# OpenDrift/opendrift

Hardware: AMD Instinct MI355X
Metric: particle-steps/sec (RK4, 3D interp) (higher is better)
Workload: dtype f64; 1 GPU; C3: OceanDrift 3D, synthetic ROMS-shaped z-level grid 1024x1024x12 (u,v,w,K), RK4 + vertical_mixing(60 s) + vertical_advection; particles_per_gpu=10000000, particles_total=10000000, stage_math=fast, spin_up_steps=200, block_every=0, inputs=resident in HBM, parallelism=particle-sharded x1, field block broadcast once per time level

## Files before the change

opendrift_amd/csrc/odr_kernels.hip.h:

```cpp
#pragma once
#include <hip/hip_runtime.h>
#include <rocrand/rocrand_kernel.h>
#include "odr_field.hip.h"

namespace odr {

#ifndef ODR_BLOCK
#define ODR_BLOCK 256
#endif
constexpr int BLOCK = ODR_BLOCK;
#ifndef ODR_POLAR_WAVES
#define ODR_POLAR_WAVES 3
#endif
#ifndef ODR_POLAR_STEP_WAVES
#define ODR_POLAR_STEP_WAVES 2
#endif
#define ODR_STEP_WAVES(PROJ) ((PROJ) == PROJ_LATLONG ? ODR_LATLONG_WAVES : ((PROJ) == PROJ_EXT ? 1 : ODR_POLAR_STEP_WAVES))
#ifndef ODR_LATLONG_WAVES
#define ODR_LATLONG_WAVES 1
#endif
#define ODR_WAVES(PROJ) ((PROJ) == PROJ_LATLONG ? ODR_LATLONG_WAVES : ((PROJ) == PROJ_EXT ? 1 : ODR_POLAR_WAVES))

__device__ __forceinline__ long long pid() {
  const unsigned nb = gridDim.x, b = blockIdx.x, per = nb >> 3, rem = nb & 7u, x = b & 7u, j = b >> 3;
// ... 259 lines not shown
    r.x = rad * ((kq == 2u || kq == 3u) ? -s1 : s1);
    r.y = rad * ((kq == 1u || kq == 2u) ? -c1 : c1);
  }
  return r;
#endif
}

constexpr unsigned long long RNG_OFF_NOISE_UNIFORM = 64, RNG_OFF_NOISE_STAGE = 128;
struct StageNoise {
  int on, rng_mode, ncomp;
  int sm;
  double std_n, std_u;
  const double *main, *stage;
  unsigned long long seed, step;
};
__device__ __forceinline__ void add_f32_f64(float &u, float &v, double nx, double ny) {
  u = (float)__dadd_rn((double)u, nx);
  v = (float)__dadd_rn((double)v, ny);
}
__device__ __forceinline__ void add_current_noise(const StageNoise &N, int call, long long i, long long n, int id,
                                                  float &u, float &v) {
  if (N.rng_mode == 1) {
    const double *a = call == 0 ? N.main : N.stage + (size_t)(call - 1) * (size_t)N.ncomp * (size_t)n;
    int c = 0;
    if (N.std_n > 0) { add_f32_f64(u, v, a[i], a[(size_t)n + i]); c = 2; }
    if (N.std_u > 0) add_f32_f64(u, v, a[(size_t)c * (size_t)n + i], a[(size_t)(c + 1) * (size_t)n + i]);
  } else {
    const unsigned long long off = RNG_OFF_NOISE + (call == 0 ? 4ull * (unsigned)VAR_U : RNG_OFF_NOISE_STAGE + 8ull * (unsigned)call);
    if (N.std_n > 0) {
      const double2 g = rng_normal2(rng_block(N.seed, id, N.step, off));
      add_f32_f64(u, v, g.x * N.std_n, g.y * N.std_n);
    }
    if (N.std_u > 0) {
      const double2 q = rng_uniform2(rng_block(N.seed, id, N.step, off + (call == 0 ? RNG_OFF_NOISE_UNIFORM : 4ull)));
      add_f32_f64(u, v, fma(2.0 * N.std_u, q.x, -N.std_u), fma(2.0 * N.std_u, q.y, -N.std_u));
    }
  }
}

#ifndef ODR_MIX_ROUNDS
#define ODR_MIX_ROUNDS 10
#endif
template <int ROUNDS>
__device__ __forceinline__ uint4 philox4x32(uint4 c, unsigned k0, unsigned k1) {
#pragma unroll
  for (int r = 0; r < ROUNDS; ++r) {
    const unsigned long long p0 = (unsigned long long)0xD2511F53u * c.x, p1 = (unsigned long long)0xCD9E8D57u * c.z;
    c = make_uint4((unsigned)(p1 >> 32) ^ c.y ^ k0, (unsigned)p1, (unsigned)(p0 >> 32) ^ c.w ^ k1, (unsigned)p0);
    k0 += 0x9E3779B9u; k1 += 0xBB67AE85u;
  }
  return c;
}
struct MixKey { unsigned k0, k1, step_lo, tag, id; };
__device__ __forceinline__ MixKey mix_key(unsigned long long seed, unsigned long long step, int id) {
  MixKey K;
  K.k0 = (unsigned)seed; K.k1 = (unsigned)(seed >> 32);
  K.step_lo = (unsigned)step; K.tag = 0x4D495856u ^ (unsigned)(step >> 32); K.id = (unsigned)id;
  return K;
}
__device__ __forceinline__ uint4 mix_block(const MixKey &K, unsigned b) {
  return philox4x32<ODR_MIX_ROUNDS>(make_uint4(b, K.step_lo, K.id, K.tag), K.k0, K.k1);
}
__device__ __forceinline__ unsigned mix_word(const uint4 &q, unsigned k) {
  const unsigned lo = ((q.x & 255u) << 16) | ((q.y & 255u) << 8) | (q.z & 255u);
  return k == 0 ? q.x >> 8 : (k == 1 ? q.y >> 8 : (k == 2 ? q.z >> 8 : (k == 3 ? q.w >> 8 : lo)));
}
__device__ __forceinline__ unsigned mix_draw(const MixKey &K, uint4 &q, int it, bool primed = false) {
  const unsigned b = (unsigned)it / 5u, k = (unsigned)it - 5u * b;
  if (k == 0 && !(primed && it == 0)) q = mix_block(K, b);
  return mix_word(q, k);
}
__device__ __forceinline__ double mix_uniform(const MixKey &K, uint4 &q, int it, bool primed = false) {
  return ((double)mix_draw(K, q, it, primed) + 0.5) * 5.9604644775390625e-08;
}
__device__ __forceinline__ double mix_R_of(unsigned x) {
  return (double)((int)(2u * x + 1u) - (1 << 24)) * 5.9604644775390625e-08;
}
constexpr int AUX_KMEMBER = 8;
struct VMixDesc {
  int sid, nzp, geo_slot;
  unsigned kstride;
  const float *kb, *ka;
  double wgt;
  float Kfb, pad2;
  const unsigned long long *guard;
};

struct VMixRT {
  static constexpr bool STATIC = false;
  __host__ __device__ static constexpr int proj_kind(int k) { return k; }
  __host__ __device__ static constexpr int lon_mode(int m) { return m; }
  __host__ __device__ static constexpr int mod360_x(int m) { return m; }
  __host__ __device__ static constexpr int nzp(int n, int ) { return n; }
  __host__ __device__ static constexpr bool uniform_z(bool u) { return u; }
  __host__ __device__ static constexpr int rng_mode(int m) { return m; }
  __host__ __device__ static constexpr int mix_at_surface(int m) { return m; }
  __host__ __device__ static constexpr int sf_action(int a) { return a; }
  __host__ __device__ static constexpr int vadv(int v) { return v; }
  __host__ __device__ static constexpr int ntimes(int n) { return n; }
  __host__ __device__ static constexpr unsigned kstride(unsigned b, int ) { return b; }
  __device__ static void proj_fwd(const DevProj &p, double lon, double lat, double &x, double &y) { proj_fwd_rt(p, lon, lat, x, y); }
};
struct VMixC3 {
  static constexpr bool STATIC = true;
  __host__ __device__ static constexpr int proj_kind(int) { return PROJ_LATLONG; }
  __host__ __device__ static constexpr int lon_mode(int) { return 1; }
  __host__ __device__ static constexpr int mod360_x(int) { return 0; }
  __host__ __device__ static constexpr int nzp(int, int NL) { return NL; }
  __host__ __device__ static constexpr bool uniform_z(bool) { return false; }
  __host__ __device__ static constexpr int rng_mode(int) { return 0; }
  __host__ __device__ static constexpr int mix_at_surface(int) { return 0; }
  __host__ __device__ static constexpr int sf_action(int) { return 1; }
  __host__ __device__ static constexpr int vadv(int) { return 0; }
  __host__ __device__ static constexpr int ntimes(int) { return 10; }
  __host__ __device__ static constexpr unsigned kstride(unsigned, int NQ) { return 16u * (unsigned)NQ; }
  __device__ static void proj_fwd(const DevProj &, double lon, double lat, double &x, double &y) { x = lon; y = lat; }
};

struct VMixC3Rec : VMixC3 {
  __host__ __device__ static constexpr unsigned kstride(unsigned b, int ) { return b; }
};

template <int NQ, bool TL, class VM, class HOOK>
__device__ __forceinline__ void vmix_col_fill(const DevSource &s, const VMixDesc &D, double lon, double lat, double *Kp,
                                              int tid, HOOK &&hook) {
  const double Kfb = (double)D.Kfb;
  double x, y;
  const int lon_mode = VM::lon_mode(s.lon_mode);
  if (lon_mode == 1) lon = np_mod(lon + 180.0, 360.0) - 180.0;
  else if (lon_mode == 2) lon = np_mod(lon, 360.0);
  VM::proj_fwd(s.proj, lon, lat, x, y);
  const bool cov = x >= s.xmin && x <= s.xmax && y >= s.ymin && y <= s.ymax;
  if (VM::mod360_x(s.mod360_x)) x = np_mod(x, 360.0);
  const DevBlock &bb = s.slot[D.geo_slot];
  const double xi = __dmul_rn(div_cr(x - bb.x0, bb.xspan, bb.ixspan), (double)(bb.nx - 1));
  const double yi = __dmul_rn(div_cr(y - bb.y0, bb.yspan, bb.iyspan), (double)(bb.ny - 1));
  const int ny = bb.ny, nx = bb.nx;
  const Axis ay = axis_fp(yi, ny), ax = axis_fp(xi, nx);
  const double ty = ay.t, tx = ax.t, wy0 = 1 - ty, wx0 = 1 - tx, wgt = D.wgt;
  const unsigned recb = VM::kstride(D.kstride, NQ);
  const unsigned r0 = __umul24((unsigned)ay.i0, (unsigned)nx), r1 = __umul24((unsigned)ay.i1, (unsigned)nx);
  const unsigned o00 = cov ? __umul24(r0 + (unsigned)ax.i0, recb) : 0u, o01 = cov ? __umul24(r0 + (unsigned)ax.i1, recb) : 0u;
  const unsigned o10 = cov ? __umul24(r1 + (unsigned)ax.i0, recb) : 0u, o11 = cov ? __umul24(r1 + (unsigned)ax.i1, recb) : 0u;
  const float *kb = D.kb, *ka = TL ? D.ka : D.kb;
  const double w00 = wy0 * wx0, w01 = wy0 * tx, w10 = ty * wx0, w11 = ty * tx;
#pragma unroll
  for (int q = 0; q < NQ; ++q) {
    if (VM::STATIC && q > 0) __builtin_amdgcn_sched_barrier(0);
    const F4 b00 = ld_off<F4>(kb, o00 + 16u * q), b01 = ld_off<F4>(kb, o01 + 16u * q);
    const F4 b10 = ld_off<F4>(kb, o10 + 16u * q), b11 = ld_off<F4>(kb, o11 + 16u * q);
    F4 a00, a01, a10, a11;
    if (TL) {
      a00 = ld_off<F4>(ka, o00 + 16u * q); a01 = ld_off<F4>(ka, o01 + 16u * q);
      a10 = ld_off<F4>(ka, o10 + 16u * q); a11 = ld_off<F4>(ka, o11 + 16u * q);
    }
    if (VM::STATIC && q > 0) __builtin_amdgcn_sched_barrier(0);
    if (q == 0) hook();
    double v[4];
    v[0] = (double)bilw(b00.x, b01.x, b10.x, b11.x, w00, w01, w10, w11);
    v[1] = (double)bilw(b00.y, b01.y, b10.y, b11.y, w00, w01, w10, w11);
    v[2] = (double)bilw(b00.z, b01.z, b10.z, b11.z, w00, w01, w10, w11);
    v[3] = (double)bilw(b00.w, b01.w, b10.w, b11.w, w00, w01, w10, w11);
    if (TL) {
      double w[4];
      w[0] = (double)bilw(a00.x, a01.x, a10.x, a11.x, w00, w01, w10, w11);
      w[1] = (double)bilw(a00.y, a01.y, a10.y, a11.y, w00, w01, w10, w11);
      w[2] = (double)bilw(a00.z, a01.z, a10.z, a11.z, w00, w01, w10, w11);
      w[3] = (double)bilw(a00.w, a01.w, a10.w, a11.w, w00, w01, w10, w11);
#pragma unroll
      for (int j = 0; j < 4; ++j) v[j] = __dadd_rn(__dmul_rn(v[j], 1 - wgt), __dmul_rn(w[j], wgt));
    }
#pragma unroll
    for (int j = 0; j < 4; ++j) Kp[(4 * q + j) * BLOCK + tid] = (cov && isfinite(v[j])) ? v[j] : Kfb;
  }
}

struct VMixArgs {
  double dt, dt_mix_cfg;
  int mix_at_surface, rng_mode, sfl, pad;
  const double *huni;
  unsigned long long seed, step;
};
struct MixRng { MixKey key; uint4 q; bool primed; };
template <class VM = VMixRT>
__device__ __forceinline__ MixRng mix_rng_begin(const VMixArgs &A, int id) {
  MixRng R;
  R.key = mix_key(A.seed, A.step, id);
  R.q = make_uint4(0u, 0u, 0u, 0u);
  R.primed = false;
  if (VM::rng_mode(A.rng_mode) == 0) {
    R.q = mix_block(R.key, 0u);
    R.primed = true;
  }
  return R;
}
template <int NQ, class VM = VMixRT>
__device__ __forceinline__ double vmix_col_walk(const DevSource &s, int nzp, const double *Kp, const double *gsh, int tid,
                                                const VMixArgs &A, long long i, long long n, int id, double z, int &moving,
                                                float Zmin, float tv, int &sf_flags, const MixRng *pre) {
  constexpr int NL = 4 * NQ;
  static_assert(!VM::STATIC || NL >= 3, "a static configuration has the three-level window inside the profile");
  const double dt = A.dt;
  const int mix_at_surface = VM::mix_at_surface(A.mix_at_surface), rng_mode = VM::rng_mode(A.rng_mode), sfl = A.sfl;
  double zm[NL - 1];
#pragma unroll
  for (int k = 0; k < NL - 1; ++k) zm[k] = k < nzp - 1 ? s.zmid[k] : __builtin_inf();
  const bool uniform_z = VM::uniform_z(s.vg_uniform != 0);
  const double gd0 = s.vg_d[0], gi0 = s.vg_id[0], gd1 = s.vg_d[1], gi1 = s.vg_id[1], gd2 = s.vg_d[2], gi2 = s.vg_id[2];
  const double sgn = dt > 0 ? 1.0 : (dt < 0 ? -1.0 : 0.0);
  const double dt_mix = A.dt_mix_cfg * sgn;
  const int ntimes = VM::ntimes(abs((int)(dt / dt_mix)));
  const double r = 1.0 / 3, ir = 1.0 / r;
  double wstep = __dmul_rn(__dmul_rn((double)tv, dt_mix), (double)moving);
  const MixKey st = mix_key(A.seed, A.step, id);
  uint4 u4 = make_uint4(0u, 0u, 0u, 0u);
  bool primed = false;
  if (pre) { u4 = pre->q; primed = pre->primed; }
  auto level_terms = [&](auto edges, int zl, double &dk_dt, double &sg) {
    constexpr int E = decltype(edges)::value;
    const double Kz = Kp[zl * BLOCK + tid];
    double gK;
    if ((E & 1) && zl == 0) gK = div_cr(Kp[BLOCK + tid] - Kz, gd0, gi0);
    else if ((E & 2) && zl == nzp - 1) gK = div_cr(Kz - Kp[(nzp - 2) * BLOCK + tid], gd1, gi1);
    else if (uniform_z) gK = div_cr(Kp[(zl + 1) * BLOCK + tid] - Kp[(zl - 1) * BLOCK + tid], gd2, gi2);
    else
      gK = __dadd_rn(__dadd_rn(__dmul_rn(gsh[zl], Kp[(zl - 1) * BLOCK + tid]), __dmul_rn(gsh[NL + zl], Kz)),
                     __dmul_rn(gsh[2 * NL + zl], Kp[(zl + 1) * BLOCK + tid]));
    double dK = -gK;
    if (fabs(dK) < 1e-10) dK = 0;
    dk_dt = __dmul_rn(dK, dt_mix);
    sg = sqrt(div_cr(__dmul_rn(__dmul_rn(Kz, fabs(dt_mix)), 2.0), r, ir));
  };
  using AnyLevel = std::integral_constant<int, 3>;
  int lv0;
  {
    const double d0 = -z;
    int zs = 0;
#pragma unroll
    for (int k = 0; k < NL - 1; ++k) zs += ((k & 1) ? d0 >= zm[k] : d0 > zm[k]) ? 1 : 0;
    lv0 = zs < 1 ? 1 : (zs > nzp - 2 ? nzp - 2 : zs);
    if (nzp < 3) lv0 = 1;
  }
  double c_dk[3], c_sg[3];
#pragma unroll
  for (int q = 0; q < 3; ++q) {
    const int zl = lv0 - 1 + q;
    c_dk[q] = 0; c_sg[q] = 0;
    if constexpr (VM::STATIC) {
      if (q == 0) level_terms(std::integral_constant<int, 1>(), zl, c_dk[q], c_sg[q]);
      else if (q == 1) level_terms(std::integral_constant<int, 0>(), zl, c_dk[q], c_sg[q]);
      else level_terms(std::integral_constant<int, 2>(), zl, c_dk[q], c_sg[q]);
    } else if (zl >= 0 && zl < nzp) level_terms(AnyLevel(), zl, c_dk[q], c_sg[q]);
  }
  double wb[4];
#pragma unroll
  for (int j = 0; j < 4; ++j) {
    const int k = lv0 - 2 + j;
    double b = k < 0 ? -1.0 : __builtin_inf();
    if (k >= 0 && k < nzp - 1) {
      b = gsh[3 * NL + k];
      if ((k & 1) && b > 0) b = __longlong_as_double(__double_as_longlong(b) - 1);
    }
    wb[j] = b;
  }
  for (int it0 = 0; it0 < ntimes; it0 += 5) {
  if (rng_mode == 0 && !(primed && it0 == 0)) u4 = mix_block(st, (unsigned)it0 / 5u);
#pragma unroll
  for (int k5 = 0; k5 < 5; ++k5) {
    const int it = it0 + k5;
    if (it >= ntimes) break;
    const bool surface = z == 0;
    const double d = -z;
    int q = (d > wb[1] ? 1 : 0) + (d > wb[2] ? 1 : 0);
    int zi = lv0 - 1 + q;
    if (!(d > wb[0]) || d > wb[3]) {
      zi = 0;
#pragma unroll
      for (int k = 0; k < NL - 1; ++k) zi += ((k & 1) ? d >= zm[k] : d > zm[k]) ? 1 : 0;
      q = zi - lv0 + 1;
    }
    double dKdt = q == 0 ? c_dk[0] : (q == 1 ? c_dk[1] : c_dk[2]);
    double sig = q == 0 ? c_sg[0] : (q == 1 ? c_sg[1] : c_sg[2]);
    if (q < 0 || q > 2) level_terms(AnyLevel(), zi, dKdt, sig);
    double R;
    if (rng_mode == 1) R = __dsub_rn(__dmul_rn(2.0, A.huni[(size_t)it * n + i]), 1.0);
    else R = mix_R_of(mix_word(u4, (unsigned)k5));
    z = __dsub_rn(z, __dmul_rn((double)moving, __dsub_rn(dKdt, __dmul_rn(R, sig))));
    if (z >= 0) z = -z;
    if (z < (double)Zmin && moving == 1) z = __dsub_rn((double)__fmul_rn(2.f, Zmin), z);
    z = __dadd_rn(z, wstep);
    if (!mix_at_surface && surface) z = 0.0;
    if (z > 0) z = 0.0;
    if (z < (double)Zmin) {
      const int act = VM::sf_action(sfl & 255);
      if (act == 3) sf_flags |= 2;
      else if (act) {
        z = (double)Zmin;
        if (act == 2) { sf_flags |= 1; moving = 0; wstep = 0.0; }
        else if (act == 4) { sf_flags |= 4; moving = 0; wstep = 0.0; }
        else if (act == 5 && (sf_flags & 8)) { sf_flags |= 4; moving = 0; wstep = 0.0; }
      }
    }
  }
  }
  return z;
}

__device__ __forceinline__ float pick_slot(const float (&a)[MAXG], int j) {
  float r = a[0];
#pragma unroll
  for (int k = 1; k < MAXG; ++k) {
    float v = a[k];
    asm volatile("" : "+v"(v));
    r = j == k ? v : r;
  }
  return r;
}

#ifdef ODR_TU_MISC
template <int NV>
struct GroupVars { int v[NV]; };

template <int NV>
__global__ __launch_bounds__(BLOCK) void k_env_group(const DevWorld *__restrict__ W, PView p,
                                                     GroupVars<NV> gv, double t, int record_prev) {
  long long i = (long long)blockIdx.x * BLOCK + threadIdx.x;
  if (i >= p.n) return;
  int vars[NV];
#pragma unroll
  for (int k = 0; k < NV; ++k) vars[k] = gv.v[k];
  double lon = p.lon[i], lat = p.lat[i], z = p.z[i];
  float out[NV];
  env_group<NV>(*W, vars, lon, lat, z, t, out, p.rank ? p.rank[i] : 0, W->f32pos & 1);
#pragma unroll
  for (int k = 0; k < NV; ++k) p.env[vars[k]][i] = out[k];
  if (record_prev) { p.slon[i] = lon; p.slat[i] = lat; }
}

template <int PROJ>
__global__ __launch_bounds__(BLOCK, ODR_WAVES(PROJ)) void k_env_grid(const DevWorld *__restrict__ W, PView p, EnvGroupDesc G,
                                                    int record_prev) {
  long long i = pid();
  if (i >= p.n) return;
  double lon = p.lon[i], lat = p.lat[i], z = p.z[i];
  int f32idx = 0;
  if (W->f32pos & 1) {
    lon = lon_f32class(W->src[G.sid].lon_mode, lon);
    if (PROJ == PROJ_LATLONG) f32idx = W->src[G.sid].xy_f32;
  }
  float out[MAXG];
  env_group_fast<PROJ>(*W, G, lon, lat, z, out, f32idx);
#pragma unroll
  for (int k = 0; k < MAXG; ++k)
    if (k < G.nv) G.out_ptr[k][i] = out[k];
  if (record_prev) { p.slon[i] = lon; p.slat[i] = lat; }
}

__global__ __launch_bounds__(BLOCK) void k_fill_f32(float *a, long long n, float v) {
  long long i = (long long)blockIdx.x * BLOCK + threadIdx.x;
  if (i < n) a[i] = v;
}

__global__ __launch_bounds__(BLOCK) void k_record_prev(PView p, int which) {
  long long i = (long long)blockIdx.x * BLOCK + threadIdx.x;
  if (i >= p.n) return;
  if (which == 0) { p.slon[i] = p.lon[i]; p.slat[i] = p.lat[i]; }
  else { p.plon[i] = p.lon[i]; p.plat[i] = p.lat[i]; }
}

#endif
#ifdef ODR_TU_STEP
__device__ __forceinline__ float rk4_mix(float k1, float k2, float k3, float k4) {
  float s = __fadd_rn(k1, __fmul_rn(2.0f, k2));
  s = __fadd_rn(s, __fmul_rn(2.0f, k3));
  s = __fadd_rn(s, k4);
  return div_cr_f32(s, 6.0f, 1.0f / 6.0f);
}

template <int SCHEME, bool NOISE>
__global__ __launch_bounds__(BLOCK) void k_advect(const DevWorld *__restrict__ W, PView p, double t,
                                                  double dt, float factor, StageNoise N) {
  long long i = (long long)blockIdx.x * BLOCK + threadIdx.x;
  if (i >= p.n) return;
  const int uv[2] = {VAR_U, VAR_V};
  double lon = p.lon[i], lat = p.lat[i], z = p.z[i];
  float u1 = p.env[VAR_U][i], v1 = p.env[VAR_V][i];
// ... 917 lines not shown
        zi += ((k & 1) ? d >= mid : d > mid) ? 1 : 0;
      }
    if (zi != zi_cur) {
      zi_cur = zi;
      const double Kz = Kp[zi * BLOCK + tid];
      double gK = 0;
      if (nzp >= 2) {
        if (zi == 0) gK = div_cr(Kp[BLOCK + tid] - Kz, src->vg_d[0], src->vg_id[0]);
        else if (zi == nzp - 1) {
          if (nzp == nz_full) gK = div_cr(Kz - Kp[(nzp - 2) * BLOCK + tid], src->vg_d[1], src->vg_id[1]);
          else gK = __ddiv_rn(Kz - Kp[(nzp - 2) * BLOCK + tid], src->z[nzp - 1] - src->z[nzp - 2]);
        } else if (uniform_z)
          gK = div_cr(Kp[(zi + 1) * BLOCK + tid] - Kp[(zi - 1) * BLOCK + tid], src->vg_d[2], src->vg_id[2]);
        else
          gK = __dadd_rn(__dadd_rn(__dmul_rn(gsh[zi], Kp[(zi - 1) * BLOCK + tid]), __dmul_rn(gsh[nzp + zi], Kz)),
                         __dmul_rn(gsh[2 * nzp + zi], Kp[(zi + 1) * BLOCK + tid]));
      }
      double dK = -gK;
      if (fabs(dK) < 1e-10) dK = 0;
      dKdt = __dmul_rn(dK, dt_mix);
      sig = sqrt(div_cr(__dmul_rn(__dmul_rn(Kz, fabs(dt_mix)), 2.0), r, ir));
    }
    double u01;
    if (rng_mode == 1) u01 = huni[(size_t)it * p.n + i];
    else u01 = mix_uniform(st, u4, it);
    double R = __dsub_rn(__dmul_rn(2.0, u01), 1.0);
    z = __dsub_rn(z, __dmul_rn((double)moving, __dsub_rn(dKdt, __dmul_rn(R, sig))));
    if (z >= 0) z = -z;
    if (z < (double)Zmin && moving == 1) z = __dsub_rn((double)__fmul_rn(2.f, Zmin), z);
    z = __dadd_rn(z, wstep);
    if (!mix_at_surface && surface) z = 0.0;
    if (z > 0) z = 0.0;
    if (OIL && z >= 0) z = oil.surface_wave_mixing(z, p, i, it, oa, seed, step);
    if (z < (double)Zmin) {
      const int act = sfl & 255;
      if (act == 3) sf_flags |= 2;
      else if (act) {
        z = (double)Zmin;
        if (act == 2) { sf_flags |= 1; moving = 0; wstep = 0.0; }
        else if (act == 4) { sf_flags |= 4; moving = 0; wstep = 0.0; }
        else if (act == 5 && (sf_flags & 8)) { sf_flags |= 4; moving = 0; wstep = 0.0; }
      }
    }
  }
  if (sf_flags & 1) {
    if (p.status[i] == 0) p.status[i] = sfl >> 8;
    p.moving[i] = 0;
  }
  if (sf_flags & 4) p.moving[i] = 0;
  if (sf_flags & 2) { p.lon[i] = p.plon[i]; p.lat[i] = p.plat[i]; }
  if (vadv >= 0 && (vadv ? z <= 0 : z < 0)) {
    double zz = __dadd_rn(z, __dmul_rn(__dmul_rn((double)moving, (double)p.env[VAR_W][i]), dt));
    z = zz < 0 ? zz : 0.0;
  }
  if (OIL) {
    p.tv[i] = (float)oil.W;
    p.aux[OIL_DIAMETER][i] = oil.d;
  }
  p.z[i] = z;
}

#ifndef ODR_VMIX_WAVES
#define ODR_VMIX_WAVES 6
#endif
struct VMixState { double slon, slat, z0; int moving, id; float dep, ssh, tv; };
__device__ __forceinline__ VMixState vmix_load_state(const PView &p, long long i) {
  VMixState S;
  S.slon = p.slon[i]; S.slat = p.slat[i]; S.z0 = p.z[i];
  S.moving = p.moving[i]; S.id = p.id[i];
  S.dep = p.env[VAR_DEPTH][i]; S.ssh = p.env[VAR_SSH][i]; S.tv = p.tv[i];
  return S;
}
template <int NQ, bool TL, class VM>
__device__ __forceinline__ void vmix_col_particle(const DevSource &s, const PView &p, const VMixDesc &D, const VMixArgs &A,
                                                  int vadv, long long i, double *Kp, const double *gsh, int tid, const VMixState &S) {
  const int nzp = VM::nzp(D.nzp, 4 * NQ), sfl = A.sfl;
  const double dt = A.dt;
  const double slon = S.slon, slat = S.slat, z0 = S.z0;
  int moving = S.moving;
  const float dep0 = S.dep, ssh0 = S.ssh, tv0 = S.tv;
  const int id0 = S.id;
  MixRng R0;
  R0.key = mix_key(A.seed, A.step, id0); R0.q = make_uint4(0u, 0u, 0u, 0u); R0.primed = false;
  vmix_col_fill<NQ, TL, VM>(s, D, slon, slat, Kp, tid, [&]() { R0 = mix_rng_begin<VM>(A, id0); });
  int sf_flags = VM::sf_action(sfl & 255) == 5 ? sf_species_flag(p, sfl, i) : 0;
  const float Zmin = __fmul_rn(-1.f, __fadd_rn(dep0, ssh0));
  double z = vmix_col_walk<NQ, VM>(s, nzp, Kp, gsh, tid, A, i, p.n, id0, z0, moving, Zmin, tv0, sf_flags, &R0);
  if (sf_flags & 1) {
    if (p.status[i] == 0) p.status[i] = sfl >> 8;
    p.moving[i] = 0;
  }
  if (sf_flags & 4) p.moving[i] = 0;
  if (sf_flags & 2) { p.lon[i] = p.plon[i]; p.lat[i] = p.plat[i]; }
  vadv = VM::vadv(vadv);
  if (vadv >= 0 && (vadv ? z <= 0 : z < 0)) {
    const float w0 = p.env[VAR_W][i];
    double zz = __dadd_rn(z, __dmul_rn(__dmul_rn((double)moving, (double)w0), dt));
    z = zz < 0 ? zz : 0.0;
  }
  p.z[i] = z;
}
template <int NQ, bool TL, class VM = VMixRT>
__global__ __launch_bounds__(BLOCK, ODR_VMIX_WAVES) void k_vmix_col(const DevWorld *__restrict__ W, PView p, VMixDesc D,
                                                    double dt, double dt_mix_cfg, int mix_at_surface,
                                                    int rng_mode, const double *__restrict__ huni,
                                                    unsigned long long seed, unsigned long long step,
                                                    int vadv, int sfl) {
  constexpr int NL = 4 * NQ;
  extern __shared__ __attribute__((aligned(16))) char smem[];
  const int tid = threadIdx.x;
  const DevSource &s = W->src[D.sid];
  const int nzp = VM::nzp(D.nzp, NL);
  double *Kp = (double *)smem;
  double *gsh = Kp + (size_t)NL * BLOCK;
  if (D.guard && *D.guard == 0ull) return;
  const long long i = pid();
  const bool valid = i < p.n;
  const VMixState S = vmix_load_state(p, valid ? i : 0);
  if (tid < nzp) {
    gsh[tid] = s.vg_a[tid]; gsh[NL + tid] = s.vg_b[tid]; gsh[2 * NL + tid] = s.vg_c[tid];
    gsh[3 * NL + tid] = s.zmid[tid];
  }
  __syncthreads();
  if (!valid) return;
  VMixArgs A;
  A.dt = dt; A.dt_mix_cfg = dt_mix_cfg; A.mix_at_surface = mix_at_surface; A.rng_mode = rng_mode; A.sfl = sfl; A.pad = 0;
  A.huni = huni; A.seed = seed; A.step = step;
  vmix_col_particle<NQ, TL, VM>(s, p, D, A, vadv, i, Kp, gsh, tid, S);
}

#ifndef ODR_VWIN_WAVES
#define ODR_VWIN_WAVES 5
#endif
template <bool TL>
__device__ __forceinline__ double vmix_layer(float b00, float b01, float b10, float b11, float a00, float a01, float a10, float a11,
                                             double w00, double w01, double w10, double w11, double wgt, bool cov, double Kfb) {
  double v = (double)bilw(b00, b01, b10, b11, w00, w01, w10, w11);
  if (TL) {
    const double w = (double)bilw(a00, a01, a10, a11, w00, w01, w10, w11);
    v = __dadd_rn(__dmul_rn(v, 1 - wgt), __dmul_rn(w, wgt));
  }
  return (cov && isfinite(v)) ? v : Kfb;
}
struct VMixGrad { double gd0, gi0, gd1, gi1, gd2, gi2, dt_mix; bool uniform_z; };
__device__ __forceinline__ void vmix_terms(const VMixGrad &G, const double *gsh, int nzp, int zl, double Kl, double Kz, double Kh,
                                           double &dk_dt, double &sg) {
  const double r = 1.0 / 3, ir = 1.0 / r;
  double gK;
  if (zl == 0) gK = div_cr(Kh - Kz, G.gd0, G.gi0);
  else if (zl == nzp - 1) gK = div_cr(Kz - Kl, G.gd1, G.gi1);
  else if (G.uniform_z) gK = div_cr(Kh - Kl, G.gd2, G.gi2);
  else gK = __dadd_rn(__dadd_rn(__dmul_rn(gsh[zl], Kl), __dmul_rn(gsh[nzp + zl], Kz)), __dmul_rn(gsh[2 * nzp + zl], Kh));
  double dK = -gK;
  if (fabs(dK) < 1e-10) dK = 0;
  dk_dt = __dmul_rn(dK, G.dt_mix);
  sg = sqrt(div_cr(__dmul_rn(__dmul_rn(Kz, fabs(G.dt_mix)), 2.0), r, ir));
}
template <bool TL>
__global__ __launch_bounds__(BLOCK, ODR_VWIN_WAVES) void k_vmix_win(const DevWorld *__restrict__ W, PView p, VMixDesc D,
                                                    double dt, double dt_mix_cfg, int mix_at_surface,
                                                    int rng_mode, const double *__restrict__ huni,
                                                    unsigned long long seed, unsigned long long step,
                                                    int vadv, int sfl) {
  extern __shared__ __attribute__((aligned(16))) char smem[];
  if (D.guard && *D.guard == 0ull) return;
  const int tid = threadIdx.x;
  const DevSource &s = W->src[D.sid];
  const int nzp = D.nzp;
  double *fw = (double *)smem;
  unsigned *fo = (unsigned *)(fw + 4 * BLOCK);
// ... 1424 lines not shown
```

opendrift_amd/csrc/odr_mix.hip:

```cpp
#define ODR_TU_MIX 1
#include "odr_host.h"

template <class VM>
static bool vmix_layout_matches(const DevSource &s, const VMixDesc &D, int nq, double dt, double dt_mix, int mix_at_surface,
                                int rng_mode, int sfl, int vadv) {
  const bool uz = s.vg_uniform != 0;
  const int ntimes = abs((int)(dt / (dt_mix * (dt > 0 ? 1.0 : (dt < 0 ? -1.0 : 0.0)))));
  return VM::proj_kind(s.proj.kind) == s.proj.kind && VM::lon_mode(s.lon_mode) == s.lon_mode &&
         VM::mod360_x(s.mod360_x) == s.mod360_x && VM::nzp(D.nzp, 4 * nq) == D.nzp && VM::uniform_z(uz) == uz &&
         VM::rng_mode(rng_mode) == rng_mode && VM::mix_at_surface(mix_at_surface) == mix_at_surface &&
         VM::sf_action(sfl & 255) == (sfl & 255) && VM::vadv(vadv) == vadv && VM::ntimes(ntimes) == ntimes &&
         VM::kstride(D.kstride, nq) == D.kstride;
}

int odr_vmix(odr_ctx *c, odr_particles *p, double t, double dt, double dt_mix, int mix_at_surface, int rng_mode,
             const double *huni, uint64_t step) {
  const bool guarded = c->guard_next_vmix != 0;
  c->guard_next_vmix = 0;
  const bool oil = c->oil_owner == p;
  const bool f32prof = p->profiles_f32;
  const int cut = c->vmix_levels;
  VMixDesc D;
  bool kplanes = !getenv("ODR_NO_KPLANE");
  const bool fast = !oil && !f32prof && cut <= 0 && !getenv("ODR_NO_FAST_PATH") && build_vmix_desc(c, t, D, kplanes);
  if (guarded && (rng_mode == ODR_RNG_HOST || !fast)) return 1;
  const int vadv = c->fuse_vadv;
  c->fuse_vadv = -1;
  c->oil_owner = nullptr;
  c->vmix_levels = 0;
  c->guarded_vmix = nullptr;
  p->status_epoch++;
  p->epoch++;
  REQUIRE(dt_mix > 0 && dt != 0, "bad time steps");
  if (!p->env[VAR_DEPTH]) return fail(ODR_ERR_STATE, "sea_floor_depth_below_sea_level has not been sampled");
  if (int rs = seafloor_species_slot_ok(c, p)) return rs;
  int rc = ensure_env(c, p, VAR_SSH);
  if (rc) return rc;
  if ((rc = flush_world(c))) return rc;
  if (p->n == 0) return 0;
  int nzp = 1;
  for (int k = 0; k < c->hw.nlist[VAR_KZ]; ++k) {
    const DevSource &s = c->hw.src[c->hw.list[VAR_KZ][k]];
    if (s.kind == SRC_GRID) { nzp = s.nz > 1 ? s.nz : 1; break; }
  }
  double *du = nullptr;
  if (rng_mode == ODR_RNG_HOST) {
    REQUIRE(huni, "host uniforms required in ODR_RNG_HOST mode");
    int ntimes = abs((int)(dt / (dt_mix * (dt > 0 ? 1 : -1))));
    void *s;
    size_t n = (size_t)ntimes * (size_t)p->n;
    if ((rc = scratch(c, p, sizeof(double) * n, &s))) return rc;
    du = (double *)s;
    H2D(du, huni, sizeof(double) * n);
    HIPCHK(hipStreamSynchronize(c->stream));
  }
  size_t lds = sizeof(double) * ((size_t)nzp * BLOCK + 3 * (size_t)nzp);
  dim3 g(nblk(p->n)), b(BLOCK);
  PView v = view(p);
  unsigned long long st = (unsigned long long)step;
  if (vadv >= 0 && !p->env[VAR_W]) return fail(ODR_ERR_STATE, "upward_sea_water_velocity has not been sampled");
  struct F32ProfileClass {
    odr_ctx *c;
    bool on;
    ~F32ProfileClass() { if (on) { c->hw.f32pos &= ~2; c->dirty = true; } }
  } f32bit{c, false};
  if (f32prof) { c->hw.f32pos |= 2; c->dirty = true; f32bit.on = true; if ((rc = flush_world(c))) return rc; }
  if (cut > 0) {
    REQUIRE(cut >= 2 && cut <= 255, "odr_vmix_set_profile_levels: 2 .. 255 levels");
    if (cut < nzp) nzp = cut;
  }
  const int sfl_cut = c->seafloor | ((cut > 0 ? nzp : 0) << 16);
  if (fast) {
    if (guarded) { D.guard = c->counter + 4; c->guarded_vmix = p; c->guarded_vadv = vadv; }
    const int nq = (nzp + 3) / 4;
    const bool tl = D.ka != nullptr;
    const char *wenv = getenv("ODR_VMIX_WINDOW");
    const bool win = nzp >= 3 && nzp <= BLOCK && (wenv ? atoi(wenv) != 0 : nzp > 12);
    const bool spec = !win && (nq == 2 || nq == 3) &&
                      vmix_layout_matches<VMixC3Rec>(c->hw.src[D.sid], D, nq, dt, dt_mix, mix_at_surface, rng_mode, c->seafloor, vadv) &&
                      !getenv("ODR_NO_VMIX_SPEC");
    const bool specp = spec && vmix_layout_matches<VMixC3>(c->hw.src[D.sid], D, nq, dt, dt_mix, mix_at_surface, rng_mode, c->seafloor, vadv);
    p->vmix_launches[win ? 2 : spec ? 1 : 0]++;
    p->vmix_kplane[kplanes ? 0 : 1]++;
#define VMIX_COL(NQ, VM)                                                                                          \
  do {                                                                                                            \
    size_t l2 = sizeof(double) * ((size_t)(4 * NQ) * BLOCK + 4 * (size_t)(4 * NQ));                               \
    if (tl) hipLaunchKernelGGL((k_vmix_col<NQ, true, VM>), g, b, l2, c->stream, c->dw, v, D, dt, dt_mix,          \
                               mix_at_surface, rng_mode, du, c->seed, st, vadv, c->seafloor);                                  \
    else hipLaunchKernelGGL((k_vmix_col<NQ, false, VM>), g, b, l2, c->stream, c->dw, v, D, dt, dt_mix,            \
                            mix_at_surface, rng_mode, du, c->seed, st, vadv, c->seafloor);                                     \
  } while (0)
    if (win) {
      const size_t lw = (sizeof(double) + sizeof(unsigned)) * 4 * BLOCK + sizeof(double) * 4 * (size_t)nzp;
      if (tl) hipLaunchKernelGGL((k_vmix_win<true>), g, b, lw, c->stream, c->dw, v, D, dt, dt_mix, mix_at_surface, rng_mode, du,
                                 c->seed, st, vadv, c->seafloor);
      else hipLaunchKernelGGL((k_vmix_win<false>), g, b, lw, c->stream, c->dw, v, D, dt, dt_mix, mix_at_surface, rng_mode, du,
                              c->seed, st, vadv, c->seafloor);
    }
    else if (specp && nq == 2) VMIX_COL(2, VMixC3);
    else if (specp) VMIX_COL(3, VMixC3);
    else if (spec && nq == 2) VMIX_COL(2, VMixC3Rec);
    else if (spec) VMIX_COL(3, VMixC3Rec);
    else if (nq <= 1) VMIX_COL(1, VMixRT);
    else if (nq == 2) VMIX_COL(2, VMixRT);
    else if (nq == 3) VMIX_COL(3, VMixRT);
    else if (nq == 4) VMIX_COL(4, VMixRT);
    else if (nq <= 6) VMIX_COL(6, VMixRT);
    else if (nq <= 8) VMIX_COL(8, VMixRT);
    else if (nq <= 12) VMIX_COL(12, VMixRT);
    else VMIX_COL(16, VMixRT);
#undef VMIX_COL
  } else if (oil) {
    if (nzp <= 16) hipLaunchKernelGGL((k_vmix<16, true>), g, b, lds, c->stream, c->dw, v, t, dt, dt_mix, mix_at_surface, rng_mode, du, c->seed, st, vadv, sfl_cut, c->oil);
    else if (nzp <= 32) hipLaunchKernelGGL((k_vmix<32, true>), g, b, lds, c->stream, c->dw, v, t, dt, dt_mix, mix_at_surface, rng_mode, du, c->seed, st, vadv, sfl_cut, c->oil);
    else hipLaunchKernelGGL((k_vmix<1, true>), g, b, lds, c->stream, c->dw, v, t, dt, dt_mix, mix_at_surface, rng_mode, du, c->seed, st, vadv, sfl_cut, c->oil);
  } else if (nzp <= 16) hipLaunchKernelGGL(k_vmix<16>, g, b, lds, c->stream, c->dw, v, t, dt, dt_mix, mix_at_surface, rng_mode, du, c->seed, st, vadv, sfl_cut);
  else if (nzp <= 32) hipLaunchKernelGGL(k_vmix<32>, g, b, lds, c->stream, c->dw, v, t, dt, dt_mix, mix_at_surface, rng_mode, du, c->seed, st, vadv, sfl_cut);
  else hipLaunchKernelGGL(k_vmix<1>, g, b, lds, c->stream, c->dw, v, t, dt, dt_mix, mix_at_surface, rng_mode, du, c->seed, st, vadv, sfl_cut);
  if (!fast) p->vmix_launches[2]++;
  HIPCHK(hipGetLastError());
  return 0;
}

int odr_particles_vmix_layout_stats(odr_ctx *c, odr_particles *p, uint64_t *out3) {
  REQUIRE(c && p && out3, "NULL argument");
  for (int k = 0; k < 3; ++k) out3[k] = p->vmix_launches[k];
  return 0;
}

int odr_particles_vmix_kplane_stats(odr_ctx *c, odr_particles *p, uint64_t *out2) {
  REQUIRE(c && p && out2, "NULL argument");
  out2[0] = p->vmix_kplane[0]; out2[1] = p->vmix_kplane[1];
  return 0;
}

int odr_vmix_set_profile_levels(odr_ctx *c, int32_t n) {
  REQUIRE(n == 0 || (n >= 2 && n <= 255), "bad level count %d", n);
  c->vmix_levels = n;
  return 0;
}

int odr_vmix_wind_profile(odr_ctx *c, odr_particles *p, int model, double background_diffusivity, double dt,
                          double dt_mix, int mix_at_surface, int rng_mode, const double *huni, uint64_t step) {
  c->guard_next_vmix = 0;
  p->status_epoch++;
  p->epoch++;
  REQUIRE(model == ODR_DIFFUSIVITY_LARGE1994 || model == ODR_DIFFUSIVITY_SUNDBY1983, "Unknown diffusivity model: %d", model);
  REQUIRE(dt_mix > 0 && dt != 0, "bad time steps");
  if (!p->env[VAR_DEPTH]) return fail(ODR_ERR_STATE, "sea_floor_depth_below_sea_level has not been sampled");
  int rc;
  if ((rc = seafloor_species_slot_ok(c, p))) return rc;
  for (int v : {VAR_SSH, VAR_XWIND, VAR_YWIND, VAR_MLD})
    if ((rc = ensure_env(c, p, v))) return rc;
  if ((rc = flush_world(c))) return rc;
  if (p->n == 0) return 0;
// ... 162 lines not shown
```

Baseline: 11.21 billion particle-steps/s.

## Skip loading diffusivity quads outside the particle's starting level window

In the static vertical-mixing column kernel, the starting level is now computed before the diffusivity profile is filled. Only the 4-level quads that the wavefront's three-level windows need are loaded, chosen by a ballot across the wavefront. If a particle later leaves the filled range, its state is parked in unused LDS, the missing quads are loaded, and the remaining mixing substeps are replayed on a slower generic path. The aim is to cut HBM gather traffic for the K field, at the cost of extra branching and a possible divergent replay path.

Result: no change. 11.23 billion particle-steps/s (median of 4 runs) (+0.3%).

```diff
diff --git a/opendrift_amd/csrc/odr_kernels.hip.h b/opendrift_amd/csrc/odr_kernels.hip.h
--- a/opendrift_amd/csrc/odr_kernels.hip.h
+++ b/opendrift_amd/csrc/odr_kernels.hip.h
@@ -365,7 +365,8 @@
   unsigned kstride;
   const float *kb, *ka;
   double wgt;
-  float Kfb, pad2;
+  float Kfb;
+  int fill_all;
   const unsigned long long *guard;
 };
 
@@ -404,10 +405,31 @@
   __host__ __device__ static constexpr unsigned kstride(unsigned b, int ) { return b; }
 };
 
-template <int NQ, bool TL, class VM, class HOOK>
-__device__ __forceinline__ void vmix_col_fill(const DevSource &s, const VMixDesc &D, double lon, double lat, double *Kp,
-                                              int tid, HOOK &&hook) {
-  const double Kfb = (double)D.Kfb;
+template <int NQ, class VM>
+constexpr bool vmix_qskip = VM::STATIC && NQ > 1;
+
+template <int NL>
+__device__ __forceinline__ int vmix_start_level(const double (&zm)[NL - 1], int nzp, double z) {
+  const double d0 = -z;
+  int zs = 0;
+#pragma unroll
+  for (int k = 0; k < NL - 1; ++k) zs += ((k & 1) ? d0 >= zm[k] : d0 > zm[k]) ? 1 : 0;
+  int lv0 = zs < 1 ? 1 : (zs > nzp - 2 ? nzp - 2 : zs);
+  if (nzp < 3) lv0 = 1;
+  return lv0;
+}
+__device__ __forceinline__ unsigned vmix_quads_of(int lo, int hi) { return (2u << (hi >> 2)) - (1u << (lo >> 2)); }
+__device__ __forceinline__ bool vmix_window_needs(int lv0, int nzp, int q) {
+  return lv0 - 2 <= 4 * q + 3 && lv0 + 2 >= 4 * q && nzp - 1 >= 4 * q;
+}
+__device__ __forceinline__ unsigned vmix_level_quads(int zi, int nzp) {
+  const int lo = zi - 1 > 0 ? zi - 1 : 0, hi = zi + 1 < nzp - 1 ? zi + 1 : nzp - 1;
+  return vmix_quads_of(lo, hi > lo ? hi : lo);
+}
+
+struct VMixFoot { unsigned o00, o01, o10, o11; double w00, w01, w10, w11; bool cov; };
+template <int NQ, class VM>
+__device__ __forceinline__ VMixFoot vmix_col_foot(const DevSource &s, const VMixDesc &D, double lon, double lat) {
   double x, y;
   const int lon_mode = VM::lon_mode(s.lon_mode);
   if (lon_mode == 1) lon = np_mod(lon + 180.0, 360.0) - 180.0;
@@ -420,41 +442,79 @@
   const double yi = __dmul_rn(div_cr(y - bb.y0, bb.yspan, bb.iyspan), (double)(bb.ny - 1));
   const int ny = bb.ny, nx = bb.nx;
   const Axis ay = axis_fp(yi, ny), ax = axis_fp(xi, nx);
-  const double ty = ay.t, tx = ax.t, wy0 = 1 - ty, wx0 = 1 - tx, wgt = D.wgt;
+  const double ty = ay.t, tx = ax.t, wy0 = 1 - ty, wx0 = 1 - tx;
   const unsigned recb = VM::kstride(D.kstride, NQ);
   const unsigned r0 = __umul24((unsigned)ay.i0, (unsigned)nx), r1 = __umul24((unsigned)ay.i1, (unsigned)nx);
   const unsigned o00 = cov ? __umul24(r0 + (unsigned)ax.i0, recb) : 0u, o01 = cov ? __umul24(r0 + (unsigned)ax.i1, recb) : 0u;
   const unsigned o10 = cov ? __umul24(r1 + (unsigned)ax.i0, recb) : 0u, o11 = cov ? __umul24(r1 + (unsigned)ax.i1, recb) : 0u;
+  VMixFoot F;
+  F.o00 = o00; F.o01 = o01; F.o10 = o10; F.o11 = o11;
+  F.w00 = wy0 * wx0; F.w01 = wy0 * tx; F.w10 = ty * wx0; F.w11 = ty * tx;
+  F.cov = cov;
+  return F;
+}
+struct VMixQuad { F4 b00, b01, b10, b11, a00, a01, a10, a11; };
+template <bool TL>
+__device__ __forceinline__ void vmix_quad_load(const VMixDesc &D, const VMixFoot &F, int q, VMixQuad &Q) {
   const float *kb = D.kb, *ka = TL ? D.ka : D.kb;
-  const double w00 = wy0 * wx0, w01 = wy0 * tx, w10 = ty * wx0, w11 = ty * tx;
+  Q.b00 = ld_off<F4>(kb, F.o00 + 16u * q); Q.b01 = ld_off<F4>(kb, F.o01 + 16u * q);
+  Q.b10 = ld_off<F4>(kb, F.o10 + 16u * q); Q.b11 = ld_off<F4>(kb, F.o11 + 16u * q);
+  if (TL) {
+    Q.a00 = ld_off<F4>(ka, F.o00 + 16u * q); Q.a01 = ld_off<F4>(ka, F.o01 + 16u * q);
+    Q.a10 = ld_off<F4>(ka, F.o10 + 16u * q); Q.a11 = ld_off<F4>(ka, F.o11 + 16u * q);
+  }
+}
+template <bool TL>
+__device__ __forceinline__ void vmix_quad_store(const VMixDesc &D, const VMixFoot &F, int q, const VMixQuad &Q, double *Kp, int tid) {
+  const double Kfb = (double)D.Kfb, wgt = D.wgt;
+  const double w00 = F.w00, w01 = F.w01, w10 = F.w10, w11 = F.w11;
+  double v[4];
+  v[0] = (double)bilw(Q.b00.x, Q.b01.x, Q.b10.x, Q.b11.x, w00, w01, w10, w11);
+  v[1] = (double)bilw(Q.b00.y, Q.b01.y, Q.b10.y, Q.b11.y, w00, w01, w10, w11);
+  v[2] = (double)bilw(Q.b00.z, Q.b01.z, Q.b10.z, Q.b11.z, w00, w01, w10, w11);
+  v[3] = (double)bilw(Q.b00.w, Q.b01.w, Q.b10.w, Q.b11.w, w00, w01, w10, w11);
+  if (TL) {
+    double w[4];
+    w[0] = (double)bilw(Q.a00.x, Q.a01.x, Q.a10.x, Q.a11.x, w00, w01, w10, w11);
+    w[1] = (double)bilw(Q.a00.y, Q.a01.y, Q.a10.y, Q.a11.y, w00, w01, w10, w11);
+    w[2] = (double)bilw(Q.a00.z, Q.a01.z, Q.a10.z, Q.a11.z, w00, w01, w10, w11);
+    w[3] = (double)bilw(Q.a00.w, Q.a01.w, Q.a10.w, Q.a11.w, w00, w01, w10, w11);
+#pragma unroll
+    for (int j = 0; j < 4; ++j) v[j] = __dadd_rn(__dmul_rn(v[j], 1 - wgt), __dmul_rn(w[j], wgt));
+  }
+#pragma unroll
+  for (int j = 0; j < 4; ++j) Kp[(4 * q + j) * BLOCK + tid] = (F.cov && isfinite(v[j])) ? v[j] : Kfb;
+}
+
+template <int NQ, bool TL, class VM, class HOOK>
+__device__ __forceinline__ void vmix_col_fill(const DevSource &s, const VMixDesc &D, double lon, double lat, double *Kp,
+                                              int tid, unsigned fill, HOOK &&hook) {
+  const VMixFoot F = vmix_col_foot<NQ, VM>(s, D, lon, lat);
+  bool hooked = false;
 #pragma unroll
   for (int q = 0; q < NQ; ++q) {
+    if (NQ > 1 && !(fill & (1u << q))) continue;
     if (VM::STATIC && q > 0) __builtin_amdgcn_sched_barrier(0);
-    const F4 b00 = ld_off<F4>(kb, o00 + 16u * q), b01 = ld_off<F4>(kb, o01 + 16u * q);
-    const F4 b10 = ld_off<F4>(kb, o10 + 16u * q), b11 = ld_off<F4>(kb, o11 + 16u * q);
-    F4 a00, a01, a10, a11;
-    if (TL) {
-      a00 = ld_off<F4>(ka, o00 + 16u * q); a01 = ld_off<F4>(ka, o01 + 16u * q);
-      a10 = ld_off<F4>(ka, o10 + 16u * q); a11 = ld_off<F4>(ka, o11 + 16u * q);
-    }
+    VMixQuad Q;
+    vmix_quad_load<TL>(D, F, q, Q);
     if (VM::STATIC && q > 0) __builtin_amdgcn_sched_barrier(0);
-    if (q == 0) hook();
-    double v[4];
-    v[0] = (double)bilw(b00.x, b01.x, b10.x, b11.x, w00, w01, w10, w11);
-    v[1] = (double)bilw(b00.y, b01.y, b10.y, b11.y, w00, w01, w10, w11);
-    v[2] = (double)bilw(b00.z, b01.z, b10.z, b11.z, w00, w01, w10, w11);
-    v[3] = (double)bilw(b00.w, b01.w, b10.w, b11.w, w00, w01, w10, w11);
-    if (TL) {
-      double w[4];
-      w[0] = (double)bilw(a00.x, a01.x, a10.x, a11.x, w00, w01, w10, w11);
-      w[1] = (double)bilw(a00.y, a01.y, a10.y, a11.y, w00, w01, w10, w11);
-      w[2] = (double)bilw(a00.z, a01.z, a10.z, a11.z, w00, w01, w10, w11);
-      w[3] = (double)bilw(a00.w, a01.w, a10.w, a11.w, w00, w01, w10, w11);
-#pragma unroll
-      for (int j = 0; j < 4; ++j) v[j] = __dadd_rn(__dmul_rn(v[j], 1 - wgt), __dmul_rn(w[j], wgt));
-    }
-#pragma unroll
-    for (int j = 0; j < 4; ++j) Kp[(4 * q + j) * BLOCK + tid] = (cov && isfinite(v[j])) ? v[j] : Kfb;
+    if (!hooked) { hook(); hooked = true; }
+    vmix_quad_store<TL>(D, F, q, Q, Kp, tid);
+  }
+}
+template <int NQ, bool TL, class VM>
+__device__ __forceinline__ void vmix_col_complete(const DevSource &s, const VMixDesc &D, const PView &p, long long i, double *Kp,
+                                                  int tid, unsigned filled) {
+  const int zero = D.fill_all;
+  VMixDesc Dc = D;
+  Dc.geo_slot += zero;
+  const VMixFoot F = vmix_col_foot<NQ, VM>((&s)[zero], Dc, p.slon[i], p.slat[i]);
+#pragma unroll 1
+  for (int q = 0; q < NQ; ++q) {
+    if (filled & (1u << q)) continue;
+    VMixQuad Q;
+    vmix_quad_load<TL>(D, F, q, Q);
+    vmix_quad_store<TL>(D, F, q, Q, Kp, tid);
   }
 }
 
@@ -477,17 +537,16 @@
   }
   return R;
 }
-template <int NQ, class VM = VMixRT>
-__device__ __forceinline__ double vmix_col_walk(const DevSource &s, int nzp, const double *Kp, const double *gsh, int tid,
+template <int NQ, class VM = VMixRT, class COMPLETE>
+__device__ __forceinline__ double vmix_col_walk(const DevSource &s, int nzp, double *Kp, const double *gsh, int tid,
                                                 const VMixArgs &A, long long i, long long n, int id, double z, int &moving,
-                                                float Zmin, float tv, int &sf_flags, const MixRng *pre) {
+                                                float Zmin, float tv, int &sf_flags, const MixRng *pre,
+                                                const double (&zm)[4 * NQ - 1], int lv0, unsigned filled, COMPLETE &&complete) {
   constexpr int NL = 4 * NQ;
+  constexpr bool QSKIP = vmix_qskip<NQ, VM>;
   static_assert(!VM::STATIC || NL >= 3, "a static configuration has the three-level window inside the profile");
   const double dt = A.dt;
   const int mix_at_surface = VM::mix_at_surface(A.mix_at_surface), rng_mode = VM::rng_mode(A.rng_mode), sfl = A.sfl;
-  double zm[NL - 1];
-#pragma unroll
-  for (int k = 0; k < NL - 1; ++k) zm[k] = k < nzp - 1 ? s.zmid[k] : __builtin_inf();
   const bool uniform_z = VM::uniform_z(s.vg_uniform != 0);
   const double gd0 = s.vg_d[0], gi0 = s.vg_id[0], gd1 = s.vg_d[1], gi1 = s.vg_id[1], gd2 = s.vg_d[2], gi2 = s.vg_id[2];
   const double sgn = dt > 0 ? 1.0 : (dt < 0 ? -1.0 : 0.0);
@@ -515,15 +574,6 @@
     sg = sqrt(div_cr(__dmul_rn(__dmul_rn(Kz, fabs(dt_mix)), 2.0), r, ir));
   };
   using AnyLevel = std::integral_constant<int, 3>;
-  int lv0;
-  {
-    const double d0 = -z;
-    int zs = 0;
-#pragma unroll
-    for (int k = 0; k < NL - 1; ++k) zs += ((k & 1) ? d0 >= zm[k] : d0 > zm[k]) ? 1 : 0;
-    lv0 = zs < 1 ? 1 : (zs > nzp - 2 ? nzp - 2 : zs);
-    if (nzp < 3) lv0 = 1;
-  }
   double c_dk[3], c_sg[3];
 #pragma unroll
   for (int q = 0; q < 3; ++q) {
@@ -546,28 +596,11 @@
     }
     wb[j] = b;
   }
-  for (int it0 = 0; it0 < ntimes; it0 += 5) {
-  if (rng_mode == 0 && !(primed && it0 == 0)) u4 = mix_block(st, (unsigned)it0 / 5u);
-#pragma unroll
-  for (int k5 = 0; k5 < 5; ++k5) {
-    const int it = it0 + k5;
-    if (it >= ntimes) break;
-    const bool surface = z == 0;
-    const double d = -z;
-    int q = (d > wb[1] ? 1 : 0) + (d > wb[2] ? 1 : 0);
-    int zi = lv0 - 1 + q;
-    if (!(d > wb[0]) || d > wb[3]) {
-      zi = 0;
-#pragma unroll
-      for (int k = 0; k < NL - 1; ++k) zi += ((k & 1) ? d >= zm[k] : d > zm[k]) ? 1 : 0;
-      q = zi - lv0 + 1;
-    }
-    double dKdt = q == 0 ? c_dk[0] : (q == 1 ? c_dk[1] : c_dk[2]);
-    double sig = q == 0 ? c_sg[0] : (q == 1 ? c_sg[1] : c_sg[2]);
-    if (q < 0 || q > 2) level_terms(AnyLevel(), zi, dKdt, sig);
-    double R;
-    if (rng_mode == 1) R = __dsub_rn(__dmul_rn(2.0, A.huni[(size_t)it * n + i]), 1.0);
-    else R = mix_R_of(mix_word(u4, (unsigned)k5));
+  auto draw = [&](int it, unsigned k) {
+    if (rng_mode == 1) return __dsub_rn(__dmul_rn(2.0, A.huni[(size_t)it * n + i]), 1.0);
+    return mix_R_of(mix_word(u4, k));
+  };
+  auto advance = [&](bool surface, double dKdt, double sig, double R) {
     z = __dsub_rn(z, __dmul_rn((double)moving, __dsub_rn(dKdt, __dmul_rn(R, sig))));
     if (z >= 0) z = -z;
     if (z < (double)Zmin && moving == 1) z = __dsub_rn((double)__fmul_rn(2.f, Zmin), z);
@@ -584,7 +617,63 @@
         else if (act == 5 && (sf_flags & 8)) { sf_flags |= 4; moving = 0; wstep = 0.0; }
       }
     }
-  }
+  };
+  auto level_of = [&](double d, auto table) {
+    int zi = 0;
+#pragma unroll
+    for (int k = 0; k < NL - 1; ++k) {
+      const double b = decltype(table)::value ? (k < nzp - 1 ? gsh[3 * NL + k] : __builtin_inf()) : zm[k];
+      zi += ((k & 1) ? d >= b : d > b) ? 1 : 0;
+    }
+    return zi;
+  };
+  int left = -1;
+  const unsigned park = QSKIP ? (unsigned)__builtin_ctz(~filled | (1u << NQ)) : 0u;
+  auto parked = [&](int j) -> double & { return Kp[(4 * (park < (unsigned)NQ ? park : 0u) + j) * BLOCK + tid]; };
+  for (int it0 = 0; it0 < ntimes; it0 += 5) {
+  if (rng_mode == 0 && !(primed && it0 == 0)) u4 = mix_block(st, (unsigned)it0 / 5u);
+#pragma unroll
+  for (int k5 = 0; k5 < 5; ++k5) {
+    const int it = it0 + k5;
+    if (it >= ntimes) break;
+    const bool surface = z == 0;
+    const double d = -z;
+    int q = (d > wb[1] ? 1 : 0) + (d > wb[2] ? 1 : 0);
+    int zi = lv0 - 1 + q;
+    if (!(d > wb[0]) || d > wb[3]) {
+      zi = level_of(d, std::false_type());
+      q = zi - lv0 + 1;
+    }
+    double dKdt = q == 0 ? c_dk[0] : (q == 1 ? c_dk[1] : c_dk[2]);
+    double sig = q == 0 ? c_sg[0] : (q == 1 ? c_sg[1] : c_sg[2]);
+    if (q < 0 || q > 2) {
+      if (QSKIP && left < 0 && (vmix_level_quads(zi, nzp) & ~filled) != 0u) {
+        left = it;
+        parked(0) = z;
+        parked(1) = wstep;
+        parked(2) = __longlong_as_double((long long)(moving | (sf_flags << 1)));
+      }
+      level_terms(AnyLevel(), zi, dKdt, sig);
+    }
+    advance(surface, dKdt, sig, draw(it, (unsigned)k5));
+  }
+  }
+  if (QSKIP && left >= 0) {
+    const long long pack = __double_as_longlong(parked(2));
+    z = parked(0);
+    wstep = parked(1);
+    moving = (int)(pack & 1);
+    sf_flags = (int)(pack >> 1);
+    complete();
+#pragma unroll 1
+    for (int it = left; it < ntimes; ++it) {
+      const unsigned k = (unsigned)it % 5u;
+      if (rng_mode == 0 && (k == 0u || it == left)) u4 = mix_block(st, (unsigned)it / 5u);
+      const bool surface = z == 0;
+      double dKdt, sig;
+      level_terms(AnyLevel(), level_of(-z, std::true_type()), dKdt, sig);
+      advance(surface, dKdt, sig, draw(it, k));
+    }
   }
   return z;
 }
@@ -1668,10 +1757,30 @@
   const int id0 = S.id;
   MixRng R0;
   R0.key = mix_key(A.seed, A.step, id0); R0.q = make_uint4(0u, 0u, 0u, 0u); R0.primed = false;
-  vmix_col_fill<NQ, TL, VM>(s, D, slon, slat, Kp, tid, [&]() { R0 = mix_rng_begin<VM>(A, id0); });
+  constexpr int NL = 4 * NQ;
+  constexpr bool QSKIP = vmix_qskip<NQ, VM>;
+  double zm[NL - 1];
+  int lv0 = 1;
+  unsigned filled = (1u << NQ) - 1u;
+  if constexpr (QSKIP) {
+    double zb[NL - 1];
+#pragma unroll
+    for (int k = 0; k < NL - 1; ++k) zb[k] = k < nzp - 1 ? gsh[3 * NL + k] : __builtin_inf();
+    lv0 = vmix_start_level<NL>(zb, nzp, z0);
+    if (!D.fill_all) {
+      filled = 0u;
+#pragma unroll
+      for (int q = 0; q < NQ; ++q) filled |= __ballot(vmix_window_needs(lv0, nzp, q)) != 0ull ? 1u << q : 0u;
+    }
+  }
+  vmix_col_fill<NQ, TL, VM>(s, D, slon, slat, Kp, tid, filled, [&]() { R0 = mix_rng_begin<VM>(A, id0); });
+#pragma unroll
+  for (int k = 0; k < NL - 1; ++k) zm[k] = k < nzp - 1 ? s.zmid[k] : __builtin_inf();
+  if constexpr (!QSKIP) lv0 = vmix_start_level<NL>(zm, nzp, z0);
   int sf_flags = VM::sf_action(sfl & 255) == 5 ? sf_species_flag(p, sfl, i) : 0;
   const float Zmin = __fmul_rn(-1.f, __fadd_rn(dep0, ssh0));
-  double z = vmix_col_walk<NQ, VM>(s, nzp, Kp, gsh, tid, A, i, p.n, id0, z0, moving, Zmin, tv0, sf_flags, &R0);
+  double z = vmix_col_walk<NQ, VM>(s, nzp, Kp, gsh, tid, A, i, p.n, id0, z0, moving, Zmin, tv0, sf_flags, &R0, zm, lv0, filled,
+                                   [&]() { vmix_col_complete<NQ, TL, VM>(s, D, p, i, Kp, tid, filled); });
   if (sf_flags & 1) {
     if (p.status[i] == 0) p.status[i] = sfl >> 8;
     p.moving[i] = 0;
diff --git a/opendrift_amd/csrc/odr_mix.hip b/opendrift_amd/csrc/odr_mix.hip
--- a/opendrift_amd/csrc/odr_mix.hip
+++ b/opendrift_amd/csrc/odr_mix.hip
@@ -71,6 +71,7 @@
   }
   const int sfl_cut = c->seafloor | ((cut > 0 ? nzp : 0) << 16);
   if (fast) {
+    D.fill_all = getenv("ODR_NO_VMIX_QSKIP") ? 1 : 0;
     if (guarded) { D.guard = c->counter + 4; c->guarded_vmix = p; c->guarded_vadv = vadv; }
     const int nq = (nzp + 3) / 4;
     const bool tl = D.ka != nullptr;
```
